# chrischoy/DeepGlobalRegistration

Hardware: AMD Instinct MI355X
Metric: pair registrations/sec (FCGF x2 + 1-NN + 6-D inlier net + gate + weighted Procrustes + SE(3) refinement) (higher is better)
Workload: dtype f32 results via 2 x f16 split operands (3 f16 MFMA products per MAC, f32 accumulate); k = 1 convs, kNN re-evaluation and registration in exact f32, SVD in f64

## Files before the change

### deepglobalregistration_amd/csrc/kmap.hip

```cpp
#include <string.h>

#include <algorithm>

#include "dgr_internal.h"
#include "hash.h"

constexpr int KM_THREADS = 256;

template <int D>
__device__ __forceinline__ void offset_of(int k, int ks, int ts, int32_t *delta) {
  const int half = ks >> 1;
#pragma unroll
  for (int d = 0; d < D; ++d) {
    delta[d] = ((k % ks) - half) * ts;
    k /= ks;
  }
}

template <int D>
__device__ __forceinline__ int probe(const int32_t *__restrict__ out_coords, int64_t o,
                                     const int32_t *delta, const int32_t *__restrict__ in_coords,
                                     const int32_t *__restrict__ in_table, uint32_t in_mask) {
  constexpr int NC = D + 1;
  int32_t q[NC];
  q[0] = out_coords[o * NC];
#pragma unroll
  for (int d = 0; d < D; ++d) q[1 + d] = out_coords[o * NC + 1 + d] + delta[d];
  return dgr_lookup<NC>(in_table, in_mask, in_coords, q);
}

template <int D>
__global__ void __launch_bounds__(KM_THREADS)
    kmap_search(const int32_t *__restrict__ out_coords, const int32_t *n_out_dev,
                const int32_t *__restrict__ in_coords, const int32_t *__restrict__ in_table,
                uint32_t in_mask, int ks, int ts_in, int RB, int64_t n_cap, int32_t *__restrict__ hits,
                int32_t *__restrict__ block_counts, int KW, uint32_t *mask_out, uint32_t *mask_in) {
  __shared__ int wave_cnt[KM_THREADS / 64];
  const int rb = blockIdx.x, k = blockIdx.y;
  const int n_out = *n_out_dev;
  if (rb * KM_THREADS >= n_out) {
    if (threadIdx.x == 0) block_counts[(int64_t)k * RB + rb] = 0;
    return;
  }
  int32_t delta[D];
  offset_of<D>(k, ks, ts_in, delta);
  const int64_t o = (int64_t)rb * KM_THREADS + threadIdx.x;
  int hit = -1;
  if (o < n_out) {
    hit = probe<D>(out_coords, o, delta, in_coords, in_table, in_mask);
    hits[(int64_t)k * n_cap + o] = hit;
    if (hit >= 0) {
      atomicOr(&mask_out[o * KW + (k >> 5)], 1u << (k & 31));
      if (mask_in) atomicOr(&mask_in[(int64_t)hit * KW + (k >> 5)], 1u << (k & 31));
    }
  }
  unsigned long long m = __ballot(hit >= 0);
  if ((threadIdx.x & 63) == 0) wave_cnt[threadIdx.x >> 6] = __popcll(m);
  __syncthreads();
  if (threadIdx.x == 0) {
    int s = 0;
#pragma unroll
    for (int w = 0; w < KM_THREADS / 64; ++w) s += wave_cnt[w];
    block_counts[(int64_t)k * RB + rb] = s;
  }
}

__device__ __forceinline__ int mask_rank(const uint32_t *__restrict__ m, int k) {
  int r = 0;
  const int w = k >> 5;
  for (int i = 0; i < w; ++i) r += __popc(m[i]);
  return r + __popc(m[w] & ((1u << (k & 31)) - 1u));
}

__global__ void mask_count_kernel(const uint32_t *__restrict__ mask, int KW, const int32_t *n_dev, int64_t n_cap,
                                  int32_t *__restrict__ cnt, unsigned short *__restrict__ wpre = nullptr) {
  const int64_t r = (int64_t)blockIdx.x * blockDim.x + threadIdx.x;
  if (r >= n_cap) return;
  int c = 0;
  if (r < *n_dev)
    for (int i = 0; i < KW; ++i) {
      if (wpre) wpre[r * KW + i] = (unsigned short)c;
      c += __popc(mask[r * KW + i]);
    }
  cnt[r] = c;
}
constexpr int KM_MC_JOBS = 8;
struct MaskCountJobs {
  const uint32_t *mask[KM_MC_JOBS];
  const int32_t *n_dev[KM_MC_JOBS];
  long long n_cap[KM_MC_JOBS];
  int32_t *cnt[KM_MC_JOBS];
  unsigned short *wpre[KM_MC_JOBS];
};
template <int KW>
__global__ void mask_count_multi(MaskCountJobs J) {
  const int m = blockIdx.y;
  const int64_t r = (int64_t)blockIdx.x * blockDim.x + threadIdx.x;
  if (r >= J.n_cap[m]) return;
  int c = 0;
  if (r < *J.n_dev[m]) {
    uint32_t w[KW];
#pragma unroll
    for (int i = 0; i < KW; ++i) w[i] = J.mask[m][r * KW + i];
#pragma unroll
    for (int i = 0; i < KW; ++i) {
      J.wpre[m][r * KW + i] = (unsigned short)c;
      c += __popc(w[i]);
    }
  }
  J.cnt[m][r] = c;
}
__device__ __forceinline__ int mask_rank_pre(const uint32_t *__restrict__ m, const unsigned short *__restrict__ pre, int k) {
  return pre[k >> 5] + __popc(m[k >> 5] & ((1u << (k & 31)) - 1u));
}


__device__ __forceinline__ unsigned long long hit_pack(int k, int64_t o, int64_t in) {
  return ((unsigned long long)k << 54) | ((unsigned long long)o << 27) | (unsigned long long)in;
}
constexpr int KM_REGION = 512;
constexpr int KM_JOBS6 = 8;
struct HitList {
  unsigned long long *recs;
  int32_t *wave_count;
  int region;
};
__device__ __forceinline__ void hit_begin(volatile int *cur) {
  if ((threadIdx.x & 63) == 0) cur[threadIdx.x >> 6] = 0;
}
__device__ __forceinline__ int64_t hit_slots(int n, const HitList &h, volatile int *cur, int wave_id) {
  const unsigned long long act = __ballot(1), two = __ballot(n == 2);
  const int lane = threadIdx.x & 63, w = threadIdx.x >> 6;
  const unsigned long long below = (1ull << lane) - 1ull;
  int base = 0;
  if (lane == __ffsll((long long)act) - 1) {
    base = cur[w];
    const int need = __popcll(act) + __popcll(two);
    if (base >= 0 && base + need <= h.region) {
      cur[w] = base + need;
    } else {
      cur[w] = -1;
      base = -1;
    }
  }
  base = __builtin_amdgcn_readfirstlane(base);
  if (base < 0) return -1;
  return (int64_t)wave_id * h.region + base + __popcll(act & below) + __popcll(two & below);
}
__device__ __forceinline__ void hit_end(const HitList &h, volatile int *cur, int wave_id) {
  if ((threadIdx.x & 63) == 0) h.wave_count[wave_id] = cur[threadIdx.x >> 6];
}

struct PrunedArgs {
  const int32_t *out_coords, *n_out_dev;
  const int4 *out_order;
  int64_t n_cap;
  DgrHalfBuckets hb;
  int ts_in, symmetric;
};
template <class Emit>
__device__ __forceinline__ void pruned_search6(const PrunedArgs &a, int64_t t, Emit &&emit) {
  const int NJ = a.symmetric ? 14 : 27;
  const int ts_in = a.ts_in;
  const int ja = (int)(t / a.n_cap);
  const int64_t p = t - (int64_t)ja * a.n_cap;
  int b = -1;
  int64_t o = 0;
  int c4 = 0, c5 = 0, c6 = 0;
  if (ja < NJ && p < *a.n_out_dev) {
    const int4 me = a.out_order[p];
    o = me.w; c4 = me.x; c5 = me.y; c6 = me.z;
    const int32_t *co = a.out_coords + o * 7;
    int32_t q[4];
    q[0] = co[0];
    q[1] = co[1] + ((ja % 3) - 1) * ts_in;
    q[2] = co[2] + (((ja / 3) % 3) - 1) * ts_in;
    q[3] = co[3] + ((ja / 9) - 1) * ts_in;
    b = dgr_lookup<4>(a.hb.table, a.hb.mask, a.hb.bkeys, q);
  }
  const int beg = b >= 0 ? a.hb.start[b] : 0, end = b >= 0 ? a.hb.start[b + 1] : 0;
  for (int p0 = beg; p0 < end; p0 += 4) {
    int4 e[4];
#pragma unroll
    for (int u = 0; u < 4; ++u) e[u] = a.hb.second[min(p0 + u, end - 1)];
#pragma unroll
    for (int u = 0; u < 4; ++u) {
      if (p0 + u >= end) break;
      const int d4 = e[u].x - c4, d5 = e[u].y - c5, d6 = e[u].z - c6;
      if (abs(d4) <= ts_in && abs(d5) <= ts_in && abs(d6) <= ts_in) {
        const int k = ja + 27 * ((d4 / ts_in + 1) + 3 * (d5 / ts_in + 1) + 9 * (d6 / ts_in + 1));
        if (a.symmetric && ja == 13 && k > 364) continue;
        emit(k, o, e[u].w);
      }
    }
  }
}

struct Bits6Jobs {
  PrunedArgs pa[KM_JOBS6];
  uint32_t *mask_out[KM_JOBS6], *mask_in[KM_JOBS6];
  HitList hl[KM_JOBS6];
  int blocks[KM_JOBS6];
};
__global__ void __launch_bounds__(KM_THREADS)
    kmap_bits_pruned6(Bits6Jobs J, int KW) {
  __shared__ int hit_cur[KM_THREADS / 64];
  const int jm = blockIdx.y;
  if ((int)blockIdx.x >= J.blocks[jm]) return;
  const PrunedArgs a = J.pa[jm];
  uint32_t *const mask_out = J.mask_out[jm], *const mask_in = J.mask_in[jm];
  const HitList hl = J.hl[jm];
  hit_begin(hit_cur);
  const int wid = (int)(blockIdx.x * (KM_THREADS / 64) + (threadIdx.x >> 6));
  pruned_search6(a, (int64_t)blockIdx.x * KM_THREADS + threadIdx.x, [&](int k, int64_t o, int in) {
    atomicOr(&mask_out[o * KW + (k >> 5)], 1u << (k & 31));
    const int km = 728 - k;
    if (a.symmetric) {
      if (km != k) atomicOr(&mask_out[(int64_t)in * KW + (km >> 5)], 1u << (km & 31));
    } else if (mask_in) {
      atomicOr(&mask_in[(int64_t)in * KW + (k >> 5)], 1u << (k & 31));
    }
    const int n = (a.symmetric && km != k) ? 2 : 1;
    const int64_t s = hit_slots(n, hl, hit_cur, wid);
    if (s >= 0) {
      hl.recs[s] = hit_pack(k, o, in);
      if (n == 2) hl.recs[s + 1] = hit_pack(km, in, o);
    }
  });
  hit_end(hl, hit_cur, wid);
}

constexpr int KM_KMAX = 736;
struct Colmask6Jobs {
  const uint32_t *mask_out[KM_JOBS6];
  const int32_t *n_out_dev[KM_JOBS6];
  int RB[KM_JOBS6];
  int4 *cell[KM_JOBS6];
  int32_t *counts[KM_JOBS6], *row_cnt[KM_JOBS6];
  unsigned short *wpre[KM_JOBS6];
};
__global__ void __launch_bounds__(KM_THREADS)
    kmap_colmask(Colmask6Jobs J, int K, int KW) {
  __shared__ unsigned long long bal[KM_THREADS / 64][KM_KMAX];
  const int jm = blockIdx.y;
  const int RB = J.RB[jm];
  if ((int)blockIdx.x >= RB) return;
  const uint32_t *__restrict__ mask_out = J.mask_out[jm];
  const int32_t *n_out_dev = J.n_out_dev[jm];
  int4 *__restrict__ cell = J.cell[jm];
  int32_t *__restrict__ counts = J.counts[jm], *__restrict__ row_cnt = J.row_cnt[jm];
  unsigned short *__restrict__ wpre = J.wpre[jm];
  const int rb = blockIdx.x;
  const int lane = threadIdx.x & 63, wave = threadIdx.x >> 6;
  const int n_out = *n_out_dev;
  const int64_t o = (int64_t)rb * KM_THREADS + threadIdx.x;
  int row_pairs = 0;
  constexpr int KW_MAX = (KM_KMAX + 31) / 32;
  uint32_t words[KW_MAX];
#pragma unroll
  for (int w = 0; w < KW_MAX; ++w) words[w] = (w < KW && o < n_out) ? mask_out[o * KW + w] : 0u;
#pragma unroll
  for (int w = 0; w < KW_MAX; ++w) {
    if (w < KW) {
      const uint32_t word = words[w];
      if (o < n_out) wpre[o * KW + w] = (unsigned short)row_pairs;
      row_pairs += __popc(word);
      unsigned long long mine = 0;
#pragma unroll
      for (int b = 0; b < 32; ++b) {
        const unsigned long long m = __ballot((word >> b) & 1u);
        if (lane == b) mine = m;
      }
      if (lane < 32 && 32 * w + lane < KM_KMAX) bal[wave][32 * w + lane] = mine;
    }
  }
  if (o < n_out) row_cnt[o] = row_pairs;
  __syncthreads();
  for (int k = threadIdx.x; k < K; k += KM_THREADS) {
    int run = 0;
#pragma unroll
    for (int g = 0; g < KM_THREADS / 64; ++g) {
      const unsigned long long m = bal[g][k];
      cell[((int64_t)rb * (KM_THREADS / 64) + g) * K + k] = make_int4((int)(m & 0xffffffffull), (int)(m >> 32), run, 0);
      run += __popcll(m);
    }
    counts[(int64_t)k * RB + rb] = run;
  }
}

struct PlaceArgs {
  int K, KW, RB;
  const uint32_t *mask_out;
  const int32_t *out_ptr;
  const int4 *cell;
  const int32_t *base;
  int32_t *pair_in, *pair_out;
  uint16_t *pair_k;
  int32_t *out_pos;
  int64_t pair_cap;
  int32_t *overflow;
  const uint32_t *mask_in;
  const int32_t *in_ptr;
  int32_t *in_pos;
  const unsigned short *wpre_out, *wpre_in;
};
__device__ __forceinline__ void place_pair(const PlaceArgs &p, int k, int64_t o, int64_t in) {
  const int64_t slot = (int64_t)p.out_ptr[o] + mask_rank_pre(p.mask_out + o * p.KW, p.wpre_out + o * p.KW, k);
  const int64_t g = o >> 6;
  const int4 c = p.cell[g * p.K + k];
  const unsigned long long cm = ((unsigned long long)(uint32_t)c.y << 32) | (uint32_t)c.x;
  const int64_t pos = (int64_t)p.base[(int64_t)k * p.RB + (g >> 2)] + c.z + __popcll(cm & ((1ull << (o & 63)) - 1ull));
  if (pos < p.pair_cap && slot < p.pair_cap) {
    p.pair_in[pos] = (int32_t)in;
    if (p.pair_out) p.pair_out[pos] = (int32_t)o;
    if (p.pair_k) p.pair_k[pos] = (uint16_t)k;
    p.out_pos[slot] = (int32_t)pos;
    if (p.mask_in) p.in_pos[p.in_ptr[in] + mask_rank_pre(p.mask_in + in * p.KW, p.wpre_in + in * p.KW, k)] = (int32_t)pos;
  } else {
    *p.overflow = 2;
  }
}

struct Place6Jobs {
  HitList h[KM_JOBS6];
  PlaceArgs p[KM_JOBS6];
  PrunedArgs replay[KM_JOBS6];
  int n_waves[KM_JOBS6], blocks[KM_JOBS6];
};
__global__ void __launch_bounds__(KM_THREADS)
    kmap_place_hits(Place6Jobs J) {
  const int jm = blockIdx.y;
  const int nblk = J.blocks[jm];
  if ((int)blockIdx.x >= nblk) return;
  const HitList h = J.h[jm];
  const PlaceArgs p = J.p[jm];
  const PrunedArgs replay = J.replay[jm];
  const int n_waves = J.n_waves[jm];
  const int lane = threadIdx.x & 63;
  for (int r = blockIdx.x * (KM_THREADS / 64) + (threadIdx.x >> 6); r < n_waves; r += nblk * (KM_THREADS / 64)) {
    const int n = h.wave_count[r];
    if (n < 0) {
      pruned_search6(replay, (int64_t)r * 64 + lane, [&](int k, int64_t o, int in) {
        place_pair(p, k, o, in);
        if (replay.symmetric && 728 - k != k) place_pair(p, 728 - k, in, o);
      });
      continue;
    }
    for (int e = lane; e < n; e += 64) {
      const unsigned long long rec = h.recs[(int64_t)r * h.region + e];
      place_pair(p, (int)(rec >> 54), (int64_t)((rec >> 27) & 0x7ffffffull), (int64_t)(rec & 0x7ffffffull));
    }
  }
}

constexpr int KM_KGROUP = 8;
__global__ void __launch_bounds__(KM_THREADS)
    kmap_fill(const int32_t *n_out_dev, int RB, int K, int64_t n_cap, const int32_t *__restrict__ hits,
              const int32_t *__restrict__ block_counts, const int32_t *__restrict__ block_base,
              int32_t *__restrict__ pair_in, int32_t *__restrict__ pair_out, int64_t pair_cap,
              int32_t *overflow, int KW, const uint32_t *__restrict__ mask_out,
              const int32_t *__restrict__ out_ptr, int32_t *__restrict__ out_pos,
              const uint32_t *__restrict__ mask_in, const int32_t *__restrict__ in_ptr,
              int32_t *__restrict__ in_pos, uint16_t *__restrict__ pair_k) {
  __shared__ int wave_cnt[2][KM_THREADS / 64];
  const int rb = blockIdx.x;
  const int n_out = *n_out_dev;
  if (rb * KM_THREADS >= n_out) return;
  const int lane = threadIdx.x & 63, wave = threadIdx.x >> 6;
  const int64_t o = (int64_t)rb * KM_THREADS + threadIdx.x;
  int parity = 0;
  for (int kk = 0; kk < KM_KGROUP; ++kk) {
    const int k = blockIdx.y * KM_KGROUP + kk;
    if (k >= K) break;
    const int64_t cell = (int64_t)k * RB + rb;
    if (block_counts[cell] == 0) continue;
    int hit = -1;
    if (o < n_out) hit = hits[(int64_t)k * n_cap + o];
    const unsigned long long m = __ballot(hit >= 0);
    if (lane == 0) wave_cnt[parity][wave] = __popcll(m);
    __syncthreads();
    if (hit >= 0) {
      int base = block_base[cell];
      for (int w = 0; w < wave; ++w) base += wave_cnt[parity][w];
      const int64_t pos = base + __popcll(m & ((1ull << lane) - 1ull));
      if (pos < pair_cap) {
        pair_in[pos] = hit;
        if (pair_out) pair_out[pos] = (int32_t)o;
        if (pair_k) pair_k[pos] = (uint16_t)k;
        out_pos[out_ptr[o] + mask_rank(mask_out + o * KW, k)] = (int32_t)pos;
        if (mask_in) in_pos[in_ptr[hit] + mask_rank(mask_in + (int64_t)hit * KW, k)] = (int32_t)pos;
      } else {
        *overflow = 2;
      }
    }
    parity ^= 1;
  }
}

constexpr int KM_MAXJOBS = 8;
struct FinalizeJobs {
  const int32_t *base[KM_MAXJOBS], *total[KM_MAXJOBS];
  int32_t *rule_ptr[KM_MAXJOBS], *tile_ptr[KM_MAXJOBS];
  int4 *desc[KM_MAXJOBS];
  long long tile_cap[KM_MAXJOBS];
  int K[KM_MAXJOBS], RB[KM_MAXJOBS];
};
__global__ void __launch_bounds__(1024) kmap_finalize(FinalizeJobs j) {
  __shared__ int s[1024];
  const int m = blockIdx.x, K = j.K[m], RB = j.RB[m];
  const int32_t *block_base = j.base[m];
  const int k = threadIdx.x;
  int start = 0, end = 0;
  if (k < K) {
    start = block_base[(int64_t)k * RB];
    end = (k + 1 < K) ? block_base[(int64_t)(k + 1) * RB] : *j.total[m];
    j.rule_ptr[m][k] = start;
    if (k == K - 1) j.rule_ptr[m][K] = end;
  }
  const int tiles = (end - start + DGR_TILE_M - 1) / DGR_TILE_M;
  s[k] = tiles;
  __syncthreads();
  for (int d = 1; d < 1024; d <<= 1) {
    const int v = (k >= d) ? s[k - d] : 0;
    __syncthreads();
    s[k] += v;
    __syncthreads();
  }
  if (k < K) j.tile_ptr[m][k] = s[k] - tiles;
  if (k == K - 1) j.tile_ptr[m][K] = s[k];
}

__device__ __forceinline__ void tile_desc_one(const int32_t *__restrict__ tile_ptr, const int32_t *__restrict__ rule_ptr, int K,
                                              int4 *__restrict__ desc, int64_t tile_cap, int64_t t, int tile_m) {
  if (t >= tile_cap || t >= tile_ptr[K]) return;
  int lo = 0, hi = K;
  while (hi - lo > 1) {
    const int mid = (lo + hi) >> 1;
    if (tile_ptr[mid] <= t) lo = mid; else hi = mid;
  }
  const int pstart = rule_ptr[lo] + ((int)t - tile_ptr[lo]) * tile_m;
  desc[t] = make_int4(lo, pstart, min(tile_m, rule_ptr[lo + 1] - pstart), 0);
}
__global__ void tile_desc_kernel(FinalizeJobs j) {
  const int m = blockIdx.y;
  const int64_t t = (int64_t)blockIdx.x * blockDim.x + threadIdx.x;
  tile_desc_one(j.tile_ptr[m], j.rule_ptr[m], j.K[m], j.desc[m], j.tile_cap[m], t, DGR_TILE_M);
}

static int alloc_kernel_map(DgrArena &arena, int K, int64_t n_cap, int64_t n_in_cap, int max_pairs_per_row, bool need_in_csr,
                            bool want_pair_out, bool want_pair_k, DgrKernelMap *km) {
  DGR_REQUIRE(K <= 1024, "kernel volume %d > 1024 not supported", K);
  km->K = K;
  const int64_t per_row = K < max_pairs_per_row ? K : max_pairs_per_row;
  km->pair_cap = per_row * n_cap;
  DGR_REQUIRE(km->pair_cap < (1ll << 31), "kernel map too large (%lld pairs)", (long long)km->pair_cap);
  DGR_ALLOC(km->rule_ptr, arena, int32_t, K + 1);
  DGR_ALLOC(km->tile_ptr, arena, int32_t, K + 1);
  DGR_ALLOC(km->pair_in, arena, int32_t, km->pair_cap);
  km->pair_out = nullptr;
  if (want_pair_out) DGR_ALLOC(km->pair_out, arena, int32_t, km->pair_cap);
  km->tile_cap = km->pair_cap / DGR_TILE_M + K;
  DGR_ALLOC(km->tile_desc, arena, int4, km->tile_cap);
  DGR_ALLOC(km->out_ptr, arena, int32_t, n_cap + 1);
  DGR_ALLOC(km->out_pos, arena, int32_t, km->pair_cap);
  km->pair_k = nullptr;
  if (want_pair_k) DGR_ALLOC(km->pair_k, arena, uint16_t, km->pair_cap);
  if (need_in_csr) {
    DGR_ALLOC(km->in_ptr, arena, int32_t, n_in_cap + 1);
    DGR_ALLOC(km->in_pos, arena, int32_t, km->pair_cap);
  }
  return DGR_OK;
}

static void finalize_job(FinalizeJobs &fj, int m, const int32_t *base, const int32_t *total, int K, int RB, DgrKernelMap *km) {
  fj.base[m] = base; fj.total[m] = total; fj.K[m] = K; fj.RB[m] = RB;
  fj.rule_ptr[m] = km->rule_ptr; fj.tile_ptr[m] = km->tile_ptr;
  fj.desc[m] = km->tile_desc; fj.tile_cap[m] = km->tile_cap;
}

static int build_kernel_map3(DgrArena &arena, const DgrCoordMap &in, const DgrCoordMap &out, int ks, int max_pairs_per_row,
                             bool need_in_csr, bool want_pair_out, bool want_pair_k, DgrKernelMap *km,
                             int32_t *overflow, hipStream_t stream) {
  constexpr int D = 3;
  const int K = ks * ks * ks;
  const int64_t n_cap = out.n_cap, n_in_cap = in.n_cap;
  const int RB = (int)dgr_ceil_div(n_cap, KM_THREADS);
  DGR_CHECK(alloc_kernel_map(arena, K, n_cap, n_in_cap, max_pairs_per_row, need_in_csr, want_pair_out, want_pair_k, km));
  const int KW = (K + 31) / 32;
  DgrArena::Mark mk = arena.mark();
  int32_t *counts, *base, *total;
  DGR_ALLOC(counts, arena, int32_t, (int64_t)K * RB);
  DGR_ALLOC(base, arena, int32_t, (int64_t)K * RB);
  DGR_ALLOC(total, arena, int32_t, 1);
  uint32_t *mask_out, *mask_in = nullptr;
  int32_t *cnt_out, *cnt_in = nullptr;
  {
    const size_t w_out = (size_t)(n_cap + 1) * KW, w_in = need_in_csr ? (size_t)(n_in_cap + 1) * KW : 0;
    DGR_ALLOC(mask_out, arena, uint32_t, w_out + w_in);
    if (need_in_csr) mask_in = mask_out + w_out;
    DGR_HIP_CHECK(hipMemsetAsync(mask_out, 0, (w_out + w_in) * sizeof(uint32_t), stream));
  }
  DGR_ALLOC(cnt_out, arena, int32_t, n_cap + 1);
  if (need_in_csr) DGR_ALLOC(cnt_in, arena, int32_t, n_in_cap + 1);
  int32_t *hits;
  DGR_ALLOC(hits, arena, int32_t, (int64_t)K * n_cap);
  kmap_search<D><<<dim3(RB, K), KM_THREADS, 0, stream>>>(out.coords, out.n_dev, in.coords, in.table, in.table_mask, ks,
                                                         in.ts, RB, n_cap, hits, counts, KW, mask_out, mask_in);
  DGR_LAUNCH_CHECK();
  mask_count_kernel<<<(int)dgr_ceil_div(n_cap + 1, 256), 256, 0, stream>>>(mask_out, KW, out.n_dev, n_cap + 1, cnt_out);
  if (need_in_csr)
    mask_count_kernel<<<(int)dgr_ceil_div(n_in_cap + 1, 256), 256, 0, stream>>>(mask_in, KW, in.n_dev, n_in_cap + 1, cnt_in);
  {
    const int32_t *ins[3] = {cnt_out, counts, cnt_in};
    int32_t *outs[3] = {km->out_ptr, base, km->in_ptr}, *tots[3] = {nullptr, total, nullptr};
    const int64_t ns[3] = {n_cap + 1, (int64_t)K * RB, n_in_cap + 1};
    DGR_CHECK(dgr_exclusive_scan_multi(arena, need_in_csr ? 3 : 2, ins, outs, ns, tots, stream));
  }
  FinalizeJobs fj = {};
  finalize_job(fj, 0, base, total, K, RB, km);
  kmap_finalize<<<1, 1024, 0, stream>>>(fj);
  tile_desc_kernel<<<dim3((unsigned)dgr_ceil_div(km->tile_cap, 256), 1), 256, 0, stream>>>(fj);
  kmap_fill<<<dim3(RB, (K + KM_KGROUP - 1) / KM_KGROUP), KM_THREADS, 0, stream>>>(
      out.n_dev, RB, K, n_cap, hits, counts, base, km->pair_in, km->pair_out, km->pair_cap, overflow, KW, mask_out,
      km->out_ptr, km->out_pos, mask_in, km->in_ptr, km->in_pos, km->pair_k);
  DGR_LAUNCH_CHECK();
  arena.rewind(mk);
  km->built = true;
  return DGR_OK;
}

struct Kmap6Job {
  const DgrCoordMap *in, *out;
  const DgrHalfBuckets *hb;
  const DgrHalfBuckets *hb_out;
  bool need_in_csr, want_pair_out, want_pair_k;
  DgrKernelMap *km;
};
static int build_kernel_maps6(DgrArena &arena, const Kmap6Job *jobs, int nj, int max_pairs_per_row, int32_t *overflow,
                              hipStream_t stream) {
  constexpr int K = 729, KW = (K + 31) / 32;
  DGR_REQUIRE(nj >= 1 && nj <= KM_MAXJOBS, "6-D kernel maps: %d jobs", nj);
  struct Tr {
    int RB, symmetric;
    int64_t n_cap, n_in_cap, hit_waves;
    int32_t *counts, *base, *total, *cnt_out, *cnt_in;
    uint32_t *mask_out, *mask_in;
    int4 *cell;
    HitList hl;
    unsigned short *wpre_out, *wpre_in;
  } t[KM_MAXJOBS];
  for (int m = 0; m < nj; ++m) {
    const Kmap6Job &J = jobs[m];
    t[m].n_cap = J.out->n_cap; t[m].n_in_cap = J.in->n_cap;
    DGR_REQUIRE(t[m].n_cap < (1ll << 27) && t[m].n_in_cap < (1ll << 27), "6-D kernel maps: more than 2^27 rows");
    DGR_CHECK(alloc_kernel_map(arena, K, t[m].n_cap, t[m].n_in_cap, max_pairs_per_row, J.need_in_csr, J.want_pair_out,
                               J.want_pair_k, J.km));
  }
  DgrArena::Mark mk = arena.mark();
  {
    size_t words = 0;
    for (int m = 0; m < nj; ++m)
      words += (size_t)(t[m].n_cap + 1) * KW + (jobs[m].need_in_csr ? (size_t)(t[m].n_in_cap + 1) * KW : 0) + (size_t)(t[m].n_cap + 1);
    uint32_t *pool;
    DGR_ALLOC(pool, arena, uint32_t, words);
    DGR_HIP_CHECK(hipMemsetAsync(pool, 0, words * sizeof(uint32_t), stream));
    for (int m = 0; m < nj; ++m) {
      t[m].mask_out = pool; pool += (size_t)(t[m].n_cap + 1) * KW;
      t[m].mask_in = nullptr;
      if (jobs[m].need_in_csr) { t[m].mask_in = pool; pool += (size_t)(t[m].n_in_cap + 1) * KW; }
      t[m].cnt_out = reinterpret_cast<int32_t *>(pool); pool += (size_t)(t[m].n_cap + 1);
    }
  }
  for (int m = 0; m < nj; ++m) {
    const Kmap6Job &J = jobs[m];
    Tr &r = t[m];
    r.RB = (int)dgr_ceil_div(r.n_cap, KM_THREADS);
    r.symmetric = (J.in->coords == J.out->coords && !J.need_in_csr) ? 1 : 0;
    DGR_REQUIRE(J.hb && J.hb->built && J.hb_out && J.hb_out->built, "6-D kernel map: first-half buckets missing");
    DGR_ALLOC(r.counts, arena, int32_t, (int64_t)K * r.RB);
    DGR_ALLOC(r.base, arena, int32_t, (int64_t)K * r.RB);
    DGR_ALLOC(r.total, arena, int32_t, 1);
    r.cnt_in = nullptr;
    if (J.need_in_csr) DGR_ALLOC(r.cnt_in, arena, int32_t, r.n_in_cap + 1);
    DGR_ALLOC(r.cell, arena, int4, (int64_t)r.RB * (KM_THREADS / 64) * K);
    const int64_t search_blocks = dgr_ceil_div(r.n_cap * (r.symmetric ? 14 : 27), KM_THREADS);
    r.hit_waves = search_blocks * (KM_THREADS / 64);
    r.hl.region = (J.in->ts >= 8 && r.symmetric) ? 2 * KM_REGION : KM_REGION / 2;
    DGR_REQUIRE(r.hit_waves < (1ll << 31), "6-D kernel map: too many search waves");
    DGR_ALLOC(r.hl.recs, arena, unsigned long long, r.hit_waves * r.hl.region);
    DGR_ALLOC(r.hl.wave_count, arena, int32_t, r.hit_waves);
    DGR_ALLOC(r.wpre_out, arena, unsigned short, (r.n_cap + 1) * KW);
    r.wpre_in = nullptr;
    if (J.need_in_csr) DGR_ALLOC(r.wpre_in, arena, unsigned short, (r.n_in_cap + 1) * KW);
  }
  static_assert(KM_JOBS6 >= KM_MAXJOBS, "multi-job launch tables");
  {
    Bits6Jobs bj = {};
    Colmask6Jobs cj = {};
    int max_sb = 0, max_rb = 0;
    for (int m = 0; m < nj; ++m) {
      const Kmap6Job &J = jobs[m];
      Tr &r = t[m];
      bj.pa[m] = PrunedArgs{J.out->coords, J.out->n_dev, J.hb_out->second, r.n_cap, *J.hb, J.in->ts, r.symmetric};
      bj.mask_out[m] = r.mask_out; bj.mask_in[m] = r.mask_in; bj.hl[m] = r.hl;
      bj.blocks[m] = (int)(r.hit_waves / (KM_THREADS / 64));
      max_sb = std::max(max_sb, bj.blocks[m]);
      cj.mask_out[m] = r.mask_out; cj.n_out_dev[m] = J.out->n_dev; cj.RB[m] = r.RB; cj.cell[m] = r.cell;
      cj.counts[m] = r.counts; cj.row_cnt[m] = r.cnt_out; cj.wpre[m] = r.wpre_out;
      max_rb = std::max(max_rb, r.RB);
    }
    kmap_bits_pruned6<<<dim3((unsigned)max_sb, (unsigned)nj), KM_THREADS, 0, stream>>>(bj, KW);
    kmap_colmask<<<dim3((unsigned)max_rb, (unsigned)nj), KM_THREADS, 0, stream>>>(cj, K, KW);
    {
      MaskCountJobs mj = {};
      int nm = 0;
      long long max_rows = 0;
      for (int m = 0; m < nj; ++m)
        if (jobs[m].need_in_csr) {
          mj.mask[nm] = t[m].mask_in; mj.n_dev[nm] = jobs[m].in->n_dev; mj.n_cap[nm] = t[m].n_in_cap + 1;
          mj.cnt[nm] = t[m].cnt_in; mj.wpre[nm] = t[m].wpre_in;
          max_rows = std::max(max_rows, mj.n_cap[nm]);
          ++nm;
        }
      static_assert(KM_MC_JOBS >= KM_MAXJOBS, "mask-count job table");
      if (nm) mask_count_multi<KW><<<dim3((unsigned)dgr_ceil_div(max_rows, 256), (unsigned)nm), 256, 0, stream>>>(mj);
    }
  }
  DGR_LAUNCH_CHECK();
  {
    const int32_t *ins[DGR_SCAN_MAX];
    int32_t *outs[DGR_SCAN_MAX], *tots[DGR_SCAN_MAX];
    int64_t ns[DGR_SCAN_MAX];
    int c = 0;
    for (int m = 0; m < nj; ++m) {
      ins[c] = t[m].cnt_out; outs[c] = jobs[m].km->out_ptr; tots[c] = nullptr; ns[c++] = t[m].n_cap + 1;
      ins[c] = t[m].counts; outs[c] = t[m].base; tots[c] = t[m].total; ns[c++] = (int64_t)K * t[m].RB;
      if (jobs[m].need_in_csr) { ins[c] = t[m].cnt_in; outs[c] = jobs[m].km->in_ptr; tots[c] = nullptr; ns[c++] = t[m].n_in_cap + 1; }
    }
    DGR_CHECK(dgr_exclusive_scan_multi(arena, c, ins, outs, ns, tots, stream));
  }
  FinalizeJobs fj = {};
  int64_t max_tiles = 0;
  for (int m = 0; m < nj; ++m) {
    finalize_job(fj, m, t[m].base, t[m].total, K, t[m].RB, jobs[m].km);
    max_tiles = std::max<int64_t>(max_tiles, jobs[m].km->tile_cap);
  }
  kmap_finalize<<<nj, 1024, 0, stream>>>(fj);
  tile_desc_kernel<<<dim3((unsigned)dgr_ceil_div(max_tiles, 256), nj), 256, 0, stream>>>(fj);
  {
    Place6Jobs pj = {};
    int max_pb = 0;
    for (int m = 0; m < nj; ++m) {
      const Kmap6Job &J = jobs[m];
      Tr &r = t[m];
      DgrKernelMap *km = J.km;
      pj.p[m] = PlaceArgs{K, KW, r.RB, r.mask_out, km->out_ptr, r.cell, r.base, km->pair_in, km->pair_out, km->pair_k, km->out_pos,
                          km->pair_cap, overflow, r.mask_in, km->in_ptr, km->in_pos, r.wpre_out, r.wpre_in};
      pj.replay[m] = PrunedArgs{J.out->coords, J.out->n_dev, J.hb_out->second, r.n_cap, *J.hb, J.in->ts, r.symmetric};
      pj.h[m] = r.hl;
      pj.n_waves[m] = (int)r.hit_waves;
      pj.blocks[m] = (int)std::min<int64_t>(dgr_ceil_div(r.hit_waves, KM_THREADS / 64), 16384);
      max_pb = std::max(max_pb, pj.blocks[m]);
      km->built = true;
    }
    kmap_place_hits<<<dim3((unsigned)max_pb, (unsigned)nj), KM_THREADS, 0, stream>>>(pj);
  }
  DGR_LAUNCH_CHECK();
  arena.rewind(mk);
  return DGR_OK;
}

constexpr int NBR_JOBS = 10;
struct NbrJobs {
  const int32_t *out_coords[NBR_JOBS], *n_out_dev[NBR_JOBS], *in_coords[NBR_JOBS], *in_table[NBR_JOBS];
  uint32_t in_mask[NBR_JOBS];
  int ts[NBR_JOBS];
  long long n_pad[NBR_JOBS];
  int32_t *nbr[NBR_JOBS];
};
__global__ void __launch_bounds__(KM_THREADS) nbr_search3(NbrJobs J) {
  const int jm = blockIdx.z;
  const int64_t n_pad = J.n_pad[jm];
  const int64_t o = (int64_t)blockIdx.x * KM_THREADS + threadIdx.x;
  if (o >= n_pad) return;
  int32_t *__restrict__ nbr = J.nbr[jm];
  const int kz = blockIdx.y;
  if (o >= *J.n_out_dev[jm]) {
#pragma unroll
    for (int u = 0; u < 9; ++u) nbr[(int64_t)(9 * kz + u) * n_pad + o] = -1;
    return;
  }
  const int sts = J.ts[jm];
  const int4 c = *reinterpret_cast<const int4 *>(J.out_coords[jm] + o * 4);
  int32_t q[9][4];
#pragma unroll
  for (int u = 0; u < 9; ++u) {
    q[u][0] = c.x;
    q[u][1] = c.y + ((u % 3) - 1) * sts;
    q[u][2] = c.z + ((u / 3) - 1) * sts;
    q[u][3] = c.w + (kz - 1) * sts;
  }
  int hit[9];
  dgr_lookup_many<4, 9>(J.in_table[jm], J.in_mask[jm], J.in_coords[jm], q, hit);
#pragma unroll
  for (int u = 0; u < 9; ++u) nbr[(int64_t)(9 * kz + u) * n_pad + o] = hit[u];
}

struct ClsJobs {
  const int32_t *coords[3], *n_dev[3];
  int ts[3], nb[3];
  int32_t *blk_cnt[3], *perm[3], *cls_count[3];
  long long cls_cap[3];
};
__device__ __forceinline__ int parity_class(const int32_t *coords, int64_t o, int ts) {
  const int4 c = *reinterpret_cast<const int4 *>(coords + o * 4);
  return ((c.y / ts) & 1) | (((c.z / ts) & 1) << 1) | (((c.w / ts) & 1) << 2);
}
__global__ void __launch_bounds__(KM_THREADS) cls_count_kernel(ClsJobs J) {
  __shared__ int wcnt[KM_THREADS / 64][8];
  const int l = blockIdx.y, b = blockIdx.x;
  if (b >= J.nb[l]) return;
  const int64_t o = (int64_t)b * KM_THREADS + threadIdx.x;
  const int cls = o < *J.n_dev[l] ? parity_class(J.coords[l], o, J.ts[l]) : 8;
#pragma unroll
  for (int c = 0; c < 8; ++c) {
    const unsigned long long m = __ballot(cls == c);
    if ((threadIdx.x & 63) == 0) wcnt[threadIdx.x >> 6][c] = __popcll(m);
  }
  __syncthreads();
  if (threadIdx.x < 8) {
    int n = 0;
    for (int w = 0; w < KM_THREADS / 64; ++w) n += wcnt[w][threadIdx.x];
    J.blk_cnt[l][b * 8 + threadIdx.x] = n;
  }
}
__global__ void __launch_bounds__(KM_THREADS) cls_fill_kernel(ClsJobs J) {
  __shared__ int part[KM_THREADS / 64][8], before[8], wcnt[KM_THREADS / 64][8];
  const int l = blockIdx.y, b = blockIdx.x;
  if (b >= J.nb[l]) return;
  const int lane = threadIdx.x & 63, wave = threadIdx.x >> 6;
  int acc[8] = {0, 0, 0, 0, 0, 0, 0, 0};
  for (int bb = threadIdx.x; bb < b; bb += KM_THREADS) {
    const int4 lo = *reinterpret_cast<const int4 *>(J.blk_cnt[l] + bb * 8), hi = *reinterpret_cast<const int4 *>(J.blk_cnt[l] + bb * 8 + 4);
    acc[0] += lo.x; acc[1] += lo.y; acc[2] += lo.z; acc[3] += lo.w;
    acc[4] += hi.x; acc[5] += hi.y; acc[6] += hi.z; acc[7] += hi.w;
  }
#pragma unroll
  for (int c = 0; c < 8; ++c) {
    int v = acc[c];
    for (int d = 32; d > 0; d >>= 1) v += __shfl_down(v, d, 64);
    if (lane == 0) part[wave][c] = v;
  }
  const int64_t o = (int64_t)b * KM_THREADS + threadIdx.x;
  const int cls = o < *J.n_dev[l] ? parity_class(J.coords[l], o, J.ts[l]) : 8;
  int rank = 0;
#pragma unroll
  for (int c = 0; c < 8; ++c) {
    const unsigned long long m = __ballot(cls == c);
    if (lane == 0) wcnt[wave][c] = __popcll(m);
    if (cls == c) rank = __popcll(m & ((1ull << lane) - 1ull));
  }
  __syncthreads();
  if (threadIdx.x < 8) {
    int n = 0;
    for (int w = 0; w < KM_THREADS / 64; ++w) n += part[w][threadIdx.x];
    before[threadIdx.x] = n;
    if (b == J.nb[l] - 1) {
      for (int w = 0; w < KM_THREADS / 64; ++w) n += wcnt[w][threadIdx.x];
      J.cls_count[l][threadIdx.x] = n;
    }
  }
  __syncthreads();
  if (cls < 8) {
    int pos = before[cls] + rank;
    for (int w = 0; w < wave; ++w) pos += wcnt[w][cls];
    J.perm[l][(int64_t)cls * J.cls_cap[l] + pos] = (int32_t)o;
  }
}

static int build_nbr_table(DgrArena &arena, const DgrCoordMap &in, const DgrCoordMap &out, int ts, int sign,
                           DgrNbrTable *t, NbrJobs *jobs, int *nj, int32_t *cls_count = nullptr) {
  t->K = 27;
  t->n_pad = dgr_ceil_div(out.n_cap, DGR_OS_ROWS) * DGR_OS_ROWS;
  DGR_ALLOC(t->nbr, arena, int32_t, t->n_pad * 27);
  t->perm = nullptr; t->cls_count = nullptr; t->cls_cap = 0;
  if (cls_count) {
    t->cls_cap = t->n_pad;
    t->cls_count = cls_count;
    DGR_ALLOC(t->perm, arena, int32_t, 8 * t->cls_cap);
  }
  DGR_REQUIRE(*nj < NBR_JOBS, "neighbour tables: more than %d per launch", NBR_JOBS);
  const int m = (*nj)++;
  jobs->out_coords[m] = out.coords; jobs->n_out_dev[m] = out.n_dev; jobs->in_coords[m] = in.coords;
  jobs->in_table[m] = in.table; jobs->in_mask[m] = in.table_mask; jobs->ts[m] = sign > 0 ? ts : -ts;
  jobs->n_pad[m] = t->n_pad; jobs->nbr[m] = t->nbr;
  t->built = true;
  return DGR_OK;
}
static int nbr_tables_launch(const NbrJobs &jobs, int nj, hipStream_t stream) {
  long long n_max = 0;
  for (int m = 0; m < nj; ++m) n_max = std::max(n_max, jobs.n_pad[m]);
  if (nj == 0) return DGR_OK;
  nbr_search3<<<dim3((unsigned)dgr_ceil_div(n_max, KM_THREADS), 3, (unsigned)nj), KM_THREADS, 0, stream>>>(jobs);
  DGR_LAUNCH_CHECK();
  return DGR_OK;
}

__global__ void nbr_count_kernel(const int32_t *__restrict__ nbr, int64_t n_pad, const int32_t *n_out_dev,
                                 unsigned long long *__restrict__ counts) {
  const int k = blockIdx.y;
  const int n = *n_out_dev;
  int c = 0;
  for (int64_t o = (int64_t)blockIdx.x * blockDim.x + threadIdx.x; o < n; o += (int64_t)gridDim.x * blockDim.x)
    c += nbr[(int64_t)k * n_pad + o] >= 0;
  for (int d = 32; d > 0; d >>= 1) c += __shfl_down(c, d, 64);
  if ((threadIdx.x & 63) == 0 && c) atomicAdd(&counts[k], (unsigned long long)c);
}

int dgr_nbr_counts(const DgrNbrTable &t, const int32_t *n_out_dev, int64_t counts[27]) {
  unsigned long long *dev;
  DGR_HIP_CHECK(hipMalloc((void **)&dev, 27 * sizeof(unsigned long long)));
  DGR_HIP_CHECK(hipMemset(dev, 0, 27 * sizeof(unsigned long long)));
  nbr_count_kernel<<<dim3(64, 27), 256>>>(t.nbr, t.n_pad, n_out_dev, dev);
  unsigned long long host[27];
  hipError_t e = hipMemcpy(host, dev, sizeof(host), hipMemcpyDeviceToHost);
  (void)hipFree(dev);
  DGR_HIP_CHECK(e);
  for (int k = 0; k < 27; ++k) counts[k] = (int64_t)host[k];
  return DGR_OK;
}

int dgr_build_coord_maps(DgrArena &arena, const int32_t *coords, int64_t N, DgrMapSet *ms,
                         hipStream_t stream);
int dgr_build_half_buckets(DgrArena &arena, DgrCoordMap *cm, DgrHalfBuckets *hb, int levels, int renumber_from, hipStream_t stream);

int dgr_build_maps(DgrArena &arena, const int32_t *coords, int64_t N, int D, int conv1_ks,
                   DgrMapSet *ms, hipStream_t stream, bool skip_conv1_map, bool lean, bool nbr_tables) {
  DGR_REQUIRE(D == 3 || D == 6, "D=%d not supported (the DGR path uses D=3 and D=6)", D);
  DGR_REQUIRE(conv1_ks % 2 == 1 && conv1_ks >= 1, "conv1 kernel size must be odd");
  DGR_REQUIRE(N > 0 && N < (1ll << 30), "N=%lld out of range", (long long)N);
  ms->D = D;
  ms->nc = D + 1;
  ms->conv1_ks = conv1_ks;
  if (!ms->overflow) {
    DGR_ALLOC(ms->overflow, arena, int32_t, 1);
    DGR_HIP_CHECK(hipMemsetAsync(ms->overflow, 0, sizeof(int32_t), stream));
  }
  DGR_CHECK(dgr_build_coord_maps(arena, coords, N, ms, stream));
  if (nbr_tables) {
    DGR_REQUIRE(D == 3, "neighbour tables are a D = 3 structure");
    ms->use_nbr = true;
    NbrJobs nbj = {};
    int n_nbj = 0;
    int32_t *cls;
    DGR_ALLOC(cls, arena, int32_t, 3 * 8);
    for (int l = 0; l < 4; ++l) DGR_CHECK(build_nbr_table(arena, ms->cm[l], ms->cm[l], ms->cm[l].ts, +1, &ms->nsame[l], &nbj, &n_nbj));
    for (int l = 0; l < 3; ++l) {
      DGR_CHECK(build_nbr_table(arena, ms->cm[l], ms->cm[l + 1], ms->cm[l].ts, +1, &ms->ndown[l], &nbj, &n_nbj));
      DGR_CHECK(build_nbr_table(arena, ms->cm[l + 1], ms->cm[l], ms->cm[l].ts, -1, &ms->nup[l], &nbj, &n_nbj, cls + 8 * l));
    }
    DGR_CHECK(nbr_tables_launch(nbj, n_nbj, stream));
    {
      ClsJobs cj = {};
      int max_nb = 0;
      for (int l = 0; l < 3; ++l) {
        cj.coords[l] = ms->cm[l].coords; cj.n_dev[l] = ms->cm[l].n_dev; cj.ts[l] = ms->cm[l].ts;
        cj.nb[l] = (int)dgr_ceil_div(ms->cm[l].n_cap, KM_THREADS);
        DGR_ALLOC(cj.blk_cnt[l], arena, int32_t, (int64_t)cj.nb[l] * 8);
        cj.perm[l] = ms->nup[l].perm; cj.cls_count[l] = ms->nup[l].cls_count; cj.cls_cap[l] = ms->nup[l].cls_cap;
        max_nb = std::max(max_nb, cj.nb[l]);
      }
      cls_count_kernel<<<dim3((unsigned)max_nb, 3), KM_THREADS, 0, stream>>>(cj);
      cls_fill_kernel<<<dim3((unsigned)max_nb, 3), KM_THREADS, 0, stream>>>(cj);
      DGR_LAUNCH_CHECK();
    }
    if (lean) {
      if (conv1_ks != 3 && !skip_conv1_map)
        DGR_CHECK(build_kernel_map3(arena, ms->cm[0], ms->cm[0], conv1_ks, 1024, false, false, true, &ms->conv1, ms->overflow,
                                    stream));
      return DGR_OK;
    }
  }
  const int cap_row = (D == 3) ? 1024 : 160;
  if (D == 6) {
    DGR_REQUIRE(conv1_ks == 3, "6-D kernel maps support kernel size 3 only (got %d)", conv1_ks);
    DGR_CHECK(dgr_build_half_buckets(arena, ms->cm, ms->hb, 4, 1, stream));
    Kmap6Job jobs[7];
    for (int l = 0; l < 4; ++l) jobs[l] = {&ms->cm[l], &ms->cm[l], &ms->hb[l], &ms->hb[l], false, !lean, !lean || l == 0, &ms->same[l]};
    for (int l = 0; l < 3; ++l) jobs[4 + l] = {&ms->cm[l], &ms->cm[l + 1], &ms->hb[l], &ms->hb[l + 1], true, true, !lean, &ms->down[l]};
    DGR_CHECK(build_kernel_maps6(arena, jobs, 7, cap_row, ms->overflow, stream));
    ms->conv1 = ms->same[0];
    return DGR_OK;
  }
  auto build = [&](const DgrCoordMap &in, const DgrCoordMap &out, int ks, bool rev, bool want_k, DgrKernelMap *km) -> int {
    const bool want_out = !lean || rev, want_pk = !lean || want_k;
    return build_kernel_map3(arena, in, out, ks, cap_row, rev, want_out, want_pk, km, ms->overflow, stream);
  };
  for (int l = 0; l < 4; ++l) DGR_CHECK(build(ms->cm[l], ms->cm[l], 3, false, l == 0, &ms->same[l]));
  if (conv1_ks == 3)
    ms->conv1 = ms->same[0];
  else if (!skip_conv1_map)
    DGR_CHECK(build(ms->cm[0], ms->cm[0], conv1_ks, false, true, &ms->conv1));
  for (int l = 0; l < 3; ++l) DGR_CHECK(build(ms->cm[l], ms->cm[l + 1], 3, true, false, &ms->down[l]));
  return DGR_OK;
}

struct dgr_maps {
  dgr_ctx *ctx;
  DgrArena arena;
  DgrMapSet ms;
  int32_t *coords_copy = nullptr;
  hipStream_t stream;
};

static int maps_create(dgr_ctx *ctx, const int32_t *coords, int64_t N, int D, int conv1_kernel_size, int flags,
                       dgr_maps **out, dgr_stream stream_) {
  DGR_REQUIRE(ctx && coords && out, "dgr_maps_create: NULL argument");
  DGR_REQUIRE((flags & ~DGR_MAPS_LEAN) == 0, "dgr_maps_create_ex: unknown flags 0x%x", flags);
  const bool lean = (flags & DGR_MAPS_LEAN) != 0;
  const bool skip_conv1_map = lean && D == 3;
  hipStream_t stream = (hipStream_t)stream_;
  DGR_HIP_CHECK(hipSetDevice(ctx->device));
  dgr_maps *m = new dgr_maps();
  m->ctx = ctx;
  m->stream = stream;
  int rc = DGR_OK;
  do {
    m->coords_copy = m->arena.get<int32_t>((size_t)N * (D + 1));
    if (!m->coords_copy) { rc = DGR_ENOMEM; break; }
    if (hipMemcpyAsync(m->coords_copy, coords, (size_t)N * (D + 1) * sizeof(int32_t),
                       hipMemcpyDeviceToDevice, stream) != hipSuccess) { rc = DGR_EHIP; break; }
    rc = dgr_build_maps(m->arena, m->coords_copy, N, D, conv1_kernel_size, &m->ms, stream, skip_conv1_map, lean, D == 3);
    if (rc != DGR_OK) break;
    int32_t flag = 0;
    if (hipMemcpyAsync(&flag, m->ms.overflow, sizeof(int32_t), hipMemcpyDeviceToHost, stream) != hipSuccess ||
        hipStreamSynchronize(stream) != hipSuccess) { rc = DGR_EHIP; dgr_set_error("maps sync failed"); break; }
    if (flag == 1) { dgr_set_error("duplicate coordinates in the sparse tensor input"); rc = DGR_EINVAL; break; }
    if (flag == 2) { dgr_set_error("kernel-map capacity exceeded"); rc = DGR_ENOMEM; break; }
  } while (0);
  if (rc != DGR_OK) {
    m->arena.release();
    delete m;
    return rc;
  }
  *out = m;
  return DGR_OK;
}

extern "C" int dgr_maps_create(dgr_ctx *ctx, const int32_t *coords, int64_t N, int D,
                               int conv1_kernel_size, dgr_maps **out, dgr_stream stream_) {
  return maps_create(ctx, coords, N, D, conv1_kernel_size, 0, out, stream_);
}

extern "C" int dgr_maps_create_ex(dgr_ctx *ctx, const int32_t *coords, int64_t N, int D, int conv1_kernel_size,
                                  int flags, dgr_maps **out, dgr_stream stream_) {
  return maps_create(ctx, coords, N, D, conv1_kernel_size, flags, out, stream_);
}

extern "C" void dgr_maps_destroy(dgr_maps *m) {
  if (!m) return;
// ... 210 lines not shown
```

Measured before the change: 395.6.

## Compute out_pos in dedicated row-wise kernel; store one hit record per symmetric pair

Drops the per-word prefix array for output rows and moves computation of out_pos into a new kernel. That kernel walks each row's mask bits with 8 lanes per row and a shuffle scan, so slots come out sequentially instead of through a rank lookup per pair. The hit list now stores one record per symmetric pair, and the mirrored pair is placed during replay, which halves record writes and region usage. The cost is an extra kernel launch and a second pass that rereads the mask and cell arrays.

```diff
diff --git a/deepglobalregistration_amd/csrc/kmap.hip b/deepglobalregistration_amd/csrc/kmap.hip
--- a/deepglobalregistration_amd/csrc/kmap.hip
+++ b/deepglobalregistration_amd/csrc/kmap.hip
@@ -128,14 +128,14 @@
 __device__ __forceinline__ void hit_begin(volatile int *cur) {
   if ((threadIdx.x & 63) == 0) cur[threadIdx.x >> 6] = 0;
 }
-__device__ __forceinline__ int64_t hit_slots(int n, const HitList &h, volatile int *cur, int wave_id) {
-  const unsigned long long act = __ballot(1), two = __ballot(n == 2);
+__device__ __forceinline__ int64_t hit_slot(const HitList &h, volatile int *cur, int wave_id) {
+  const unsigned long long act = __ballot(1);
   const int lane = threadIdx.x & 63, w = threadIdx.x >> 6;
   const unsigned long long below = (1ull << lane) - 1ull;
   int base = 0;
   if (lane == __ffsll((long long)act) - 1) {
     base = cur[w];
-    const int need = __popcll(act) + __popcll(two);
+    const int need = __popcll(act);
     if (base >= 0 && base + need <= h.region) {
       cur[w] = base + need;
     } else {
@@ -145,12 +145,13 @@
   }
   base = __builtin_amdgcn_readfirstlane(base);
   if (base < 0) return -1;
-  return (int64_t)wave_id * h.region + base + __popcll(act & below) + __popcll(two & below);
+  return (int64_t)wave_id * h.region + base + __popcll(act & below);
 }
 __device__ __forceinline__ void hit_end(const HitList &h, volatile int *cur, int wave_id) {
   if ((threadIdx.x & 63) == 0) h.wave_count[wave_id] = cur[threadIdx.x >> 6];
 }
 
+constexpr int KM_SCAN_W = 4;
 struct PrunedArgs {
   const int32_t *out_coords, *n_out_dev;
   const int4 *out_order;
@@ -179,12 +180,12 @@
     b = dgr_lookup<4>(a.hb.table, a.hb.mask, a.hb.bkeys, q);
   }
   const int beg = b >= 0 ? a.hb.start[b] : 0, end = b >= 0 ? a.hb.start[b + 1] : 0;
-  for (int p0 = beg; p0 < end; p0 += 4) {
-    int4 e[4];
-#pragma unroll
-    for (int u = 0; u < 4; ++u) e[u] = a.hb.second[min(p0 + u, end - 1)];
-#pragma unroll
-    for (int u = 0; u < 4; ++u) {
+  for (int p0 = beg; p0 < end; p0 += KM_SCAN_W) {
+    int4 e[KM_SCAN_W];
+#pragma unroll
+    for (int u = 0; u < KM_SCAN_W; ++u) e[u] = a.hb.second[min(p0 + u, end - 1)];
+#pragma unroll
+    for (int u = 0; u < KM_SCAN_W; ++u) {
       if (p0 + u >= end) break;
       const int d4 = e[u].x - c4, d5 = e[u].y - c5, d6 = e[u].z - c6;
       if (abs(d4) <= ts_in && abs(d5) <= ts_in && abs(d6) <= ts_in) {
@@ -220,12 +221,8 @@
     } else if (mask_in) {
       atomicOr(&mask_in[(int64_t)in * KW + (k >> 5)], 1u << (k & 31));
     }
-    const int n = (a.symmetric && km != k) ? 2 : 1;
-    const int64_t s = hit_slots(n, hl, hit_cur, wid);
-    if (s >= 0) {
-      hl.recs[s] = hit_pack(k, o, in);
-      if (n == 2) hl.recs[s + 1] = hit_pack(km, in, o);
-    }
+    const int64_t s = hit_slot(hl, hit_cur, wid);
+    if (s >= 0) hl.recs[s] = hit_pack(k, o, in);
   });
   hit_end(hl, hit_cur, wid);
 }
@@ -237,7 +234,6 @@
   int RB[KM_JOBS6];
   int4 *cell[KM_JOBS6];
   int32_t *counts[KM_JOBS6], *row_cnt[KM_JOBS6];
-  unsigned short *wpre[KM_JOBS6];
 };
 __global__ void __launch_bounds__(KM_THREADS)
     kmap_colmask(Colmask6Jobs J, int K, int KW) {
@@ -249,7 +245,6 @@
   const int32_t *n_out_dev = J.n_out_dev[jm];
   int4 *__restrict__ cell = J.cell[jm];
   int32_t *__restrict__ counts = J.counts[jm], *__restrict__ row_cnt = J.row_cnt[jm];
-  unsigned short *__restrict__ wpre = J.wpre[jm];
   const int rb = blockIdx.x;
   const int lane = threadIdx.x & 63, wave = threadIdx.x >> 6;
   const int n_out = *n_out_dev;
@@ -263,7 +258,6 @@
   for (int w = 0; w < KW_MAX; ++w) {
     if (w < KW) {
       const uint32_t word = words[w];
-      if (o < n_out) wpre[o * KW + w] = (unsigned short)row_pairs;
       row_pairs += __popc(word);
       unsigned long long mine = 0;
 #pragma unroll
@@ -288,33 +282,87 @@
   }
 }
 
+__device__ __forceinline__ int64_t pair_position(const int4 *__restrict__ cell, const int32_t *__restrict__ base, int K, int RB,
+                                                 int k, int64_t o) {
+  const int64_t g = o >> 6;
+  const int4 c = cell[g * K + k];
+  const unsigned long long cm = ((unsigned long long)(uint32_t)c.y << 32) | (uint32_t)c.x;
+  return (int64_t)base[(int64_t)k * RB + (g >> 2)] + c.z + __popcll(cm & ((1ull << (o & 63)) - 1ull));
+}
+
+constexpr int KM_OP_LANES = 8, KM_OP_WORDS = 3;
+static_assert(KM_OP_LANES * KM_OP_WORDS * 32 >= KM_KMAX, "kmap_out_pos: a row's lanes cover every offset");
+struct OutPos6Jobs {
+  const uint32_t *mask_out[KM_JOBS6];
+  const int32_t *n_out_dev[KM_JOBS6], *out_ptr[KM_JOBS6], *base[KM_JOBS6];
+  const int4 *cell[KM_JOBS6];
+  int32_t *out_pos[KM_JOBS6];
+  long long pair_cap[KM_JOBS6];
+  int RB[KM_JOBS6];
+  int32_t *overflow;
+};
+__global__ void __launch_bounds__(KM_THREADS)
+    kmap_out_pos(OutPos6Jobs J, int K, int KW) {
+  const int jm = blockIdx.y;
+  const int n_out = *J.n_out_dev[jm];
+  constexpr int ROWS = KM_THREADS / KM_OP_LANES;
+  if ((int64_t)blockIdx.x * ROWS >= n_out) return;
+  const int64_t o = (int64_t)blockIdx.x * ROWS + threadIdx.x / KM_OP_LANES;
+  const int w = threadIdx.x % KM_OP_LANES;
+  uint32_t word[KM_OP_WORDS];
+  int mine = 0;
+#pragma unroll
+  for (int i = 0; i < KM_OP_WORDS; ++i) {
+    const int wi = w * KM_OP_WORDS + i;
+    word[i] = (o < n_out && wi < KW) ? J.mask_out[jm][o * KW + wi] : 0u;
+    mine += __popc(word[i]);
+  }
+  int upto = mine;
+#pragma unroll
+  for (int d = 1; d < KM_OP_LANES; d <<= 1) {
+    const int v = __shfl_up(upto, d, KM_OP_LANES);
+    if (w >= d) upto += v;
+  }
+  if (!mine) return;
+  int64_t slot = (int64_t)J.out_ptr[jm][o] + upto - mine;
+  const int4 *__restrict__ cell = J.cell[jm];
+  const int32_t *__restrict__ base = J.base[jm];
+  int32_t *__restrict__ out_pos = J.out_pos[jm];
+  const int64_t pair_cap = J.pair_cap[jm];
+  const int RB = J.RB[jm];
+#pragma unroll
+  for (int i = 0; i < KM_OP_WORDS; ++i) {
+    uint32_t wd = word[i];
+    while (wd) {
+      const int k = 32 * (w * KM_OP_WORDS + i) + __ffs((int)wd) - 1;
+      wd &= wd - 1u;
+      const int64_t pos = pair_position(cell, base, K, RB, k, o);
+      if (pos < pair_cap && slot < pair_cap) out_pos[slot] = (int32_t)pos;
+      else *J.overflow = 2;
+      ++slot;
+    }
+  }
+}
+
 struct PlaceArgs {
   int K, KW, RB;
-  const uint32_t *mask_out;
-  const int32_t *out_ptr;
   const int4 *cell;
   const int32_t *base;
   int32_t *pair_in, *pair_out;
   uint16_t *pair_k;
-  int32_t *out_pos;
   int64_t pair_cap;
   int32_t *overflow;
   const uint32_t *mask_in;
   const int32_t *in_ptr;
   int32_t *in_pos;
-  const unsigned short *wpre_out, *wpre_in;
+  const unsigned short *wpre_in;
 };
 __device__ __forceinline__ void place_pair(const PlaceArgs &p, int k, int64_t o, int64_t in) {
-  const int64_t slot = (int64_t)p.out_ptr[o] + mask_rank_pre(p.mask_out + o * p.KW, p.wpre_out + o * p.KW, k);
-  const int64_t g = o >> 6;
-  const int4 c = p.cell[g * p.K + k];
-  const unsigned long long cm = ((unsigned long long)(uint32_t)c.y << 32) | (uint32_t)c.x;
-  const int64_t pos = (int64_t)p.base[(int64_t)k * p.RB + (g >> 2)] + c.z + __popcll(cm & ((1ull << (o & 63)) - 1ull));
-  if (pos < p.pair_cap && slot < p.pair_cap) {
+  const int64_t pos = pair_position(p.cell, p.base, p.K, p.RB, k, o);
+  if (pos < p.pair_cap) {
     p.pair_in[pos] = (int32_t)in;
     if (p.pair_out) p.pair_out[pos] = (int32_t)o;
     if (p.pair_k) p.pair_k[pos] = (uint16_t)k;
-    p.out_pos[slot] = (int32_t)pos;
     if (p.mask_in) p.in_pos[p.in_ptr[in] + mask_rank_pre(p.mask_in + in * p.KW, p.wpre_in + in * p.KW, k)] = (int32_t)pos;
   } else {
     *p.overflow = 2;
@@ -348,7 +396,10 @@
     }
     for (int e = lane; e < n; e += 64) {
       const unsigned long long rec = h.recs[(int64_t)r * h.region + e];
-      place_pair(p, (int)(rec >> 54), (int64_t)((rec >> 27) & 0x7ffffffull), (int64_t)(rec & 0x7ffffffull));
+      const int k = (int)(rec >> 54);
+      const int64_t o = (int64_t)((rec >> 27) & 0x7ffffffull), in = (int64_t)(rec & 0x7ffffffull);
+      place_pair(p, k, o, in);
+      if (replay.symmetric && 728 - k != k) place_pair(p, 728 - k, in, o);
     }
   }
 }
@@ -547,7 +598,7 @@
     uint32_t *mask_out, *mask_in;
     int4 *cell;
     HitList hl;
-    unsigned short *wpre_out, *wpre_in;
+    unsigned short *wpre_in;
   } t[KM_MAXJOBS];
   for (int m = 0; m < nj; ++m) {
     const Kmap6Job &J = jobs[m];
@@ -589,7 +640,6 @@
     DGR_REQUIRE(r.hit_waves < (1ll << 31), "6-D kernel map: too many search waves");
     DGR_ALLOC(r.hl.recs, arena, unsigned long long, r.hit_waves * r.hl.region);
     DGR_ALLOC(r.hl.wave_count, arena, int32_t, r.hit_waves);
-    DGR_ALLOC(r.wpre_out, arena, unsigned short, (r.n_cap + 1) * KW);
     r.wpre_in = nullptr;
     if (J.need_in_csr) DGR_ALLOC(r.wpre_in, arena, unsigned short, (r.n_in_cap + 1) * KW);
   }
@@ -606,7 +656,7 @@
       bj.blocks[m] = (int)(r.hit_waves / (KM_THREADS / 64));
       max_sb = std::max(max_sb, bj.blocks[m]);
       cj.mask_out[m] = r.mask_out; cj.n_out_dev[m] = J.out->n_dev; cj.RB[m] = r.RB; cj.cell[m] = r.cell;
-      cj.counts[m] = r.counts; cj.row_cnt[m] = r.cnt_out; cj.wpre[m] = r.wpre_out;
+      cj.counts[m] = r.counts; cj.row_cnt[m] = r.cnt_out;
       max_rb = std::max(max_rb, r.RB);
     }
     kmap_bits_pruned6<<<dim3((unsigned)max_sb, (unsigned)nj), KM_THREADS, 0, stream>>>(bj, KW);
@@ -648,14 +698,25 @@
   kmap_finalize<<<nj, 1024, 0, stream>>>(fj);
   tile_desc_kernel<<<dim3((unsigned)dgr_ceil_div(max_tiles, 256), nj), 256, 0, stream>>>(fj);
   {
+    OutPos6Jobs oj = {};
+    oj.overflow = overflow;
+    int64_t max_rows = 0;
+    for (int m = 0; m < nj; ++m) {
+      const Tr &r = t[m];
+      const DgrKernelMap *km = jobs[m].km;
+      oj.mask_out[m] = r.mask_out; oj.n_out_dev[m] = jobs[m].out->n_dev; oj.out_ptr[m] = km->out_ptr; oj.base[m] = r.base;
+      oj.cell[m] = r.cell; oj.out_pos[m] = km->out_pos; oj.pair_cap[m] = km->pair_cap; oj.RB[m] = r.RB;
+      max_rows = std::max(max_rows, r.n_cap);
+    }
+    kmap_out_pos<<<dim3((unsigned)dgr_ceil_div(max_rows, KM_THREADS / KM_OP_LANES), (unsigned)nj), KM_THREADS, 0, stream>>>(oj, K, KW);
     Place6Jobs pj = {};
     int max_pb = 0;
     for (int m = 0; m < nj; ++m) {
       const Kmap6Job &J = jobs[m];
       Tr &r = t[m];
       DgrKernelMap *km = J.km;
-      pj.p[m] = PlaceArgs{K, KW, r.RB, r.mask_out, km->out_ptr, r.cell, r.base, km->pair_in, km->pair_out, km->pair_k, km->out_pos,
-                          km->pair_cap, overflow, r.mask_in, km->in_ptr, km->in_pos, r.wpre_out, r.wpre_in};
+      pj.p[m] = PlaceArgs{K, KW, r.RB, r.cell, r.base, km->pair_in, km->pair_out, km->pair_k, km->pair_cap, overflow,
+                          r.mask_in, km->in_ptr, km->in_pos, r.wpre_in};
       pj.replay[m] = PrunedArgs{J.out->coords, J.out->n_dev, J.hb_out->second, r.n_cap, *J.hb, J.in->ts, r.symmetric};
       pj.h[m] = r.hl;
       pj.n_waves[m] = (int)r.hit_waves;
```

New measurement: 399.7, median of 6. 1.0% higher.
